# xuanyi-fu/xynet

Hardware: AMD Instinct MI355X
Metric: GiB/s device-resident WebSocket XOR-unmask, 64KiB frames, 1/2/4/8 GPUs (higher is better)
Workload: dtype u8; 1 GPU; config 3: 32768 x 64 KiB masked binary frames (H=14), one contiguous 2 GiB batch; decoder=lattice (k_stream_lattice), mode=fused (xyws_decode_stream: boundaries discovered on device), frames_per_gpu=32768, batch_bytes_per_gpu=2147942400, payload_bytes_per_gpu=2147483648, batch_copies=1, parallelism=shard-by-frame x1, no collective

## Files before the change

xynet_amd/_lib.py:

```python
import ctypes as C
import os
import re

PKG = os.path.dirname(os.path.abspath(__file__))
ROOT = os.path.dirname(PKG)
HEADER = os.path.join(ROOT, "include", "xyws.h")

XYWS_OK = 0
XYWS_ERR_DEVICE = -5
OPT_PARSE_ONLY = 0x1
OPT_UNMASKED_HINT = 0x2
OPT_SERIAL_SCAN = 0x4
OPT_WG256 = 0x8
OPT_TEST_LATSPEC = 0x10
OPT_TEST_LATDUMP = 0x20
OPT_LATX_NOWORK = 0x40
OPT_LATX_ONLY = 0x80
OPT_STATS = 0x100
OPT_SMALL_SEG = 0x200
OPT_LATTICE = 0x400
OPT_NO_LATDEC = 0x800
OPT_NO_DENSE0 = 0x1000
OPT_REDIRECT = 0x2000
OPT_NO_LATENTRY = 0x4000
OPT_WG1024 = 0x8000
OPT_RUNS_NOWAIT = 0x10000
OPT_NO_STORE = 0x20000
OPT_WG512 = 0x40000
OPT_DIAG = 0x80000
OPT_TEST_GIVEUP = 0x100000
OPT_NO_LATTICE = 0x200000
OPT_STEAL = 0x400000
OPT_TEST_STEAL = 0x800000
OPT_LAT_NOGATE = 0x1000000
OPT_LAT_GATE = 0x2000000
OPT_BIGSCAN = 0x4000000
OPT_LATX_NOCHK = 0x8000000
OPT_IOV_PIECES = 0x10000000
OPT_IOV_STAGE = 0x20000000
OPT_NO_BIGSCAN = 0x40000000
OPT_RUNS = 0x80000000
NSTATS = 48
ST_RUNS, ST_NONE, ST_BAD, ST_REPAIR, ST_CUT, ST_SPIN, ST_SEGS, ST_FRAMES = 0, 1, 2, 3, 4, 5, 6, 7
ST_P_WIN, ST_P_CAND, ST_P_UND, ST_P_TCOMP, ST_P_TCHECK, ST_P_TRES = 8, 9, 10, 11, 12, 13
ST_D_TENT, ST_D_TCHASE = 14, 15
ST_T_PRO, ST_T_MAIN, ST_T_WAIT, ST_T_FILL, ST_T_CHASE, ST_T_XOR = 16, 17, 18, 19, 20, 21
ST_T_TAIL, ST_T_PF, ST_T_CP = 22, 23, 24
ST_P_FILL, ST_P_SCAN, ST_P_PUB, ST_D_NOENT, ST_D_CHASE, ST_D_MISMATCH, ST_D_OVF = 25, 26, 27, 28, 29, 30, 31
ST_GIVEUP, ST_BRIDGE, ST_STEAL_REQ, ST_STEAL_ACC, ST_STEAL_SEGS = 32, 33, 34, 35, 36
ST_D_TVAL, ST_T_ROWS, ST_T_SER = 37, 38, 39
ST_P_LATTICE, ST_X_W0, ST_X_BITS, ST_X_SURV, ST_T_STRIDE = 40, 41, 42, 43, 46
LT_C_A, LT_C_C, LT_C_ADV, LT_D_FILL, LT_D_WB, LT_D_TAB, LT_D_WC = 16, 17, 18, 19, 20, 21, 22
LT_D_MASK, LT_D_WD, LT_D_ST, LT_D_WA, LT_SEGS, LT_GATE, LT_END = 23, 24, 25, 26, 27, 28, 29
R_WORDS = 32
R_H, R_W, R_S0, R_HEAD, R_OKW, R_HN, R_WN, R_CNT, R_TAIL, R_FIRST, R_F0 = 0, 1, 2, 7, 8, 9, 10, 11, 12, 13, 14
R_EFROM, R_ECNT, R_EORD, R_ECARRY, R_EP = 20, 21, 22, 23, 24
R_T0, R_T1, R_T2, R_SPLIT, R_XCC, R_NREC = 25, 26, 27, 28, 29, 30
POL_EPOCH, POL_BYTES, POL_FSMIN, POL_FSMAX, POL_DECODER, POL_WORDS = 0, 1, 2, 3, 4, 5
DEC_RUNS, DEC_RUNS512, DEC_LATTICE = 0, 2, 3
DERR_TABLE, DERR_TIMEOUT, DERR_STALE, DERR_TAG, DERR_SRC_OOB, DERR_ORPHANS = 0x1, 0x2, 0x4, 0x8, 0x100, 0x200
ERRORS = {-1: "invalid argument", -2: "HIP runtime error", -3: "device allocation failed",
          -4: "scratch capacity exceeded", -5: "device-side error", -6: "not complete yet"}


class XywsError(RuntimeError):
    def __init__(self, code, what=""):
        self.code = code
        super().__init__(f"xyws error {code} ({ERRORS.get(code, '?')}){': ' + what if what else ''}")


class Frame(C.Structure):
    _fields_ = [("frame_off", C.c_int64), ("payload_off", C.c_int64),
                ("payload_len", C.c_uint64), ("key", C.c_uint8 * 4),
                ("flags", C.c_uint8), ("hdr_len", C.c_uint8),
                ("status", C.c_uint8), ("reserved", C.c_uint8)]


class Carry(C.Structure):
    _fields_ = [("payload_remaining", C.c_uint64), ("phase", C.c_uint64),
                ("frames_total", C.c_uint64), ("key", C.c_uint8 * 4),
                ("hdr_len", C.c_uint8), ("hdr", C.c_uint8 * 14),
                ("reserved", C.c_uint8 * 21)]


class Verdict(C.Structure):
    _fields_ = [("close_code", C.c_uint16), ("peer_code", C.c_uint16), ("action", C.c_uint8),
                ("reserved", C.c_uint8 * 3)]


class Message(C.Structure):
    _fields_ = [("first_frame", C.c_uint64), ("nframes", C.c_uint64), ("out_off", C.c_uint64),
                ("length", C.c_uint64), ("status", C.c_uint32), ("opcode", C.c_uint8),
                ("reserved", C.c_uint8 * 3)]


class MsgCarry(C.Structure):
    _fields_ = [("length", C.c_uint64), ("nframes", C.c_uint64), ("first_frame", C.c_uint64),
                ("frame_remaining", C.c_uint64), ("frames_seen", C.c_uint64), ("status", C.c_uint32),
                ("opcode", C.c_uint8), ("frame_member", C.c_uint8), ("utf8_len", C.c_uint8),
                ("utf8", C.c_uint8 * 3), ("reserved", C.c_uint8 * 14)]


class ArenaResult(C.Structure):
    _fields_ = [("seq", C.c_uint64), ("offset", C.c_uint64), ("len", C.c_uint64), ("nframes", C.c_uint64),
                ("frames", C.POINTER(Frame)), ("carry", Carry)]


class Conn(C.Structure):
    _fields_ = [("buf", C.c_void_p), ("len", C.c_uint64), ("carry", C.c_void_p), ("frames", C.c_void_p),
                ("cap", C.c_uint64), ("reserved", C.c_uint64 * 3)]


class ReplyCarry(C.Structure):
    _fields_ = [("frame_remaining", C.c_uint64), ("frames_seen", C.c_uint64), ("replies_total", C.c_uint64),
                ("close_code", C.c_uint16), ("echoing", C.c_uint8), ("status", C.c_uint8),
                ("reserved", C.c_uint8 * 4)]


class ReplyConn(C.Structure):
    _fields_ = [("out", C.c_void_p), ("out_cap", C.c_uint64), ("rc", C.c_void_p), ("verdicts", C.c_void_p)]


class ReplyResult(C.Structure):
    _fields_ = [("reply_len", C.c_uint64), ("first_close", C.c_uint64), ("answered", C.c_uint32),
# ... 498 lines not shown
```

xynet_amd/csrc/xyws_lattice.h:

```cpp

constexpr uint64_t LAT_FMIN = 128;
constexpr uint64_t LAT_FMAX = 1ull << 40;
enum { LS_AGG = 1, LS_BRK = 3 };
constexpr uint32_t LAT_SLIST = 512;
constexpr uint32_t LAT_NOCLAIM = 0x7FFFFFFFu;
enum : uint64_t { RD_DONE = 0, RD_FULL = 1, RD_FROM = 2 };

template <uint32_t NT_, uint32_t SEG_>
struct lgeom {
  static constexpr uint32_t NT = NT_, SEG = SEG_;
  static constexpr uint32_t TMAX = SEG_ / LAT_FMIN + 3;
};
using G_LAT = lgeom<1024, 15 * 8 * 1024>;
using G_LAT5 = lgeom<1024, 15 * 5 * 1024>;
constexpr uint64_t LAT5_MIN_FRAME = 16384;
using G_LAT_SMALL = lgeom<64, 1024>;


template <class GA, class GB>
struct llay {
  static_assert(GA::NT == GB::NT, "one workgroup size");
  static constexpr uint32_t NT = GA::NT;
  static constexpr uint32_t SEG = GA::SEG > GB::SEG ? GA::SEG : GB::SEG;
  static constexpr uint32_t TMAX = GA::TMAX > GB::TMAX ? GA::TMAX : GB::TMAX;
};
template <class GL>
struct __attribute__((aligned(256))) lat_lds {
  cstate S0;
  uint64_t E, X0, F, kmax, c0, kbf, nseg;
  uint64_t gk;
  uint32_t na, cur, nxt, brk, quit, done_last, nsl, big, nogate;
  uint64_t sl_seg[LAT_SLIST], sl_k[LAT_SLIST];
  uint4 tab[GL::TMAX];
  alignas(256) uint8_t seg[GL::SEG + 48];
};

XYWS_DEV uint32_t lat_rel(uint64_t x, uint64_t ss) {
  if (x <= ss) return 0;
  const uint64_t d = x - ss;
  return d > 0xFFFFFFFFull ? 0xFFFFFFFFu : (uint32_t)d;
}

constexpr uint32_t LAT_GRP = 64;
XYWS_DEV uint64_t lat_grp_size(const run_params& P, uint64_t g) {
  const uint64_t a = g * LAT_GRP;
  return a >= P.nseg ? 0 : (P.nseg - a < LAT_GRP ? P.nseg - a : LAT_GRP);
}

XYWS_DEV uint64_t lat_advance(const run_params& P, uint64_t E, uint32_t lane) {
  const uint64_t w = uniform64(st_load(P.lat + LW_W));
  if (w >= P.nseg) return w;
  uint64_t w1 = w;
  {
    const uint64_t g0 = w / LAT_GRP, g = g0 + lane, gs = lat_grp_size(P, g);
    const bool full = !gs || st_load(P.lgrp + g) == gs;
    const uint64_t nf = __ballot(!full);
    const uint32_t c = nf ? (uint32_t)__builtin_ctzll(nf) : 64u;
    const uint64_t wg = (g0 + c) * LAT_GRP;
    if (wg > w1) w1 = wg < P.nseg ? wg : P.nseg;
  }
  if (w1 < P.nseg) {
    bool dec[4];
#pragma unroll
    for (uint32_t r = 0; r < 4; r++) {
      const uint64_t j = w1 + 4 * lane + r;
      dec[r] = j >= P.nseg || (st_load(P.lat + LW_STAT + j) >> 2) == E;
    }
    const uint32_t lc = !dec[0] ? 0u : !dec[1] ? 1u : !dec[2] ? 2u : !dec[3] ? 3u : 4u;
    const uint64_t nd = __ballot(lc < 4);
    uint64_t w2 = w1 + 256;
    if (nd) {
      const uint32_t f = (uint32_t)__builtin_ctzll(nd);
      w2 = w1 + 4 * f + (uint32_t)__shfl((int)lc, (int)f, 64);
    }
    w1 = w2 < P.nseg ? w2 : P.nseg;
  }
  if (w1 > w && lane == 0) __hip_atomic_fetch_max(P.lat + LW_W, w1, __ATOMIC_RELAXED, __HIP_MEMORY_SCOPE_AGENT);
  return w1;
}
XYWS_DEV void lat_wait_decided(const run_params& P, uint64_t E, uint64_t s, uint32_t lane) {
  for (uint32_t it = 0; lat_advance(P, E, lane) <= s; it++) {
    if (it >= (1u << 20)) {
      if (lane == 0) atomicOr(head_error(P), DERR_TIMEOUT);
      return;
    }
    __builtin_amdgcn_s_sleep(8);
  }
}

XYWS_DEV u32x4 lat_mask(const uint4* tab, uint32_t nent, uint32_t idx, uint32_t a) {
  const uint4 g = tab[idx];
  if (g.x <= a && a + 16u <= g.y) return u32x4{g.z, g.z, g.z, g.z};
  u32x4 m = span_key16(a, g.x, g.y, g.z);
  if (idx + 1 < nent) {
    const uint4 n = tab[idx + 1];
    if (n.x < a + 16u) m |= span_key16(a, n.x, n.y, n.z);
  }
  return m;
}

XYWS_DEV hdr_info lat_hdr(const run_params& P, const uint8_t* seg, uint32_t xr, uint64_t x) {
  const uint32_t* q = reinterpret_cast<const uint32_t*>(seg + (xr & ~3u));
  const uint32_t sh = xr & 3u, r0 = q[0], r1 = q[1], r2 = q[2], r3 = q[3], r4 = q[4];
  uint32_t w[4];
  w[0] = __builtin_amdgcn_alignbyte(r1, r0, sh);
  w[1] = __builtin_amdgcn_alignbyte(r2, r1, sh);
  w[2] = __builtin_amdgcn_alignbyte(r3, r2, sh);
  w[3] = __builtin_amdgcn_alignbyte(r4, r3, sh);
  const uint64_t room = P.hi - x;
  return parse_header_words(w, room < 16 ? (uint32_t)room : 16u);
}

XYWS_DEV __amdgpu_buffer_rsrc_t lat_rsrc(const run_params& P, uint64_t ss, uint32_t n) {
  const uint64_t top = (P.hi + 15) & ~15ull;
  const uint64_t room = top > ss ? top - ss : 0;
  return __builtin_amdgcn_make_buffer_rsrc(P.base + ss, 0, room < n ? (uint32_t)room : n, 0x00020000);
}

XYWS_DEV void write_frame(const run_params& P, uint64_t ord, uint64_t start, const hdr_info& h, uint64_t ps,
                          int32_t hdr_shift);

XYWS_DEV void lat_carried_frame(const run_params& P, const xyws_carry* cz) {
  if (!P.frames || !P.cap || cz->payload_remaining || !cz->hdr_len) return;
  const hdr_info hh = header_carried(P, cz);
  if (hh.hlen) write_frame(P, 0, P.lo, hh, P.lo + (hh.hlen - cz->hdr_len), (int32_t)cz->hdr_len);
}

template <class LL>
XYWS_DEV void lat_finish(const run_params& P, LL& L) {
  uint64_t* rd = P.lat + LW_REDIR;
  const xyws_carry* cz = P.cin_user ? P.cin_user : &k_zero_carry;
  {
    const uint32_t w = L.na == 2 ? LW_NBAIL_POL : L.na ? LW_NBAIL_HYP : L.big ? LW_NLOOP_A : LW_NLOOP_B;
    st_store(P.lat + w, st_load(P.lat + w) + 1);
  }
  if (L.na) {
    st_store(rd, RD_FULL);
  } else {
    const uint64_t b = st_load(P.lat + LW_BRK);
    const uint64_t X0 = L.X0, F = L.F, kmax = L.kmax, c0 = L.c0;
    lat_carried_frame(P, cz);
    if (b) {
      const uint64_t kb = ~b;
      const uint64_t tb = c0 + kb;
      uint64_t* rc = P.lat + LW_RCARRY;
#pragma unroll
      for (int i = 0; i < 8; i++) st_store(rc + i, 0);
      st_store(rc + 2, cz->frames_total + tb);
      st_store(rd + 1, X0 + kb * F);
      st_store(rd + 2, tb);
      st_store(rd, RD_FROM);
    } else {
      const uint64_t xl = X0 + (kmax - 1) * F;
      const hdr_info h = hdr_global(P, xl, NONE);
      uint64_t total = c0 + kmax;
      cstate S;
      if (!h.hlen) {
        S.X = xl; S.cov_ps = xl; S.cov_start = xl; S.cov_kw = 0; S.cov_key = 0; S.st = S_PARTIAL | S_NOCOV; S.pad = 0;
        total--;
      } else {
        S = frame_state(xl, h);
      }
      xyws_carry cinc;
#pragma unroll
      for (int i = 0; i < 8; i++) reinterpret_cast<uint64_t*>(&cinc)[i] = reinterpret_cast<const uint64_t*>(cz)[i];
      write_outputs(P, &cinc, total, S);
      dpol_publish(P, F, DEC_LATTICE);
      if (P.pol) {
        const uint64_t v[5] = {L.E, P.hi - P.lo, F, F, DEC_LATTICE};
#pragma unroll
        for (int i = 1; i < 5; i++) __hip_atomic_store(P.pol + i, v[i], __ATOMIC_RELAXED, __HIP_MEMORY_SCOPE_SYSTEM);
        __hip_atomic_store(P.pol, v[0], __ATOMIC_RELEASE, __HIP_MEMORY_SCOPE_SYSTEM);
      }
      st_store(rd, RD_DONE);
    }
  }
  uint32_t* cnt = reinterpret_cast<uint32_t*>(P.lat + LW_CNT);
  st_store(P.lat + LW_BRK, 0);
  st_store(P.lat + LW_W, 0);
  st_store(P.lat + LW_LOOPS, 0);
  __hip_atomic_store(cnt, 0u, __ATOMIC_RELAXED, __HIP_MEMORY_SCOPE_AGENT);
  __hip_atomic_store(cnt + 1, 0u, __ATOMIC_RELAXED, __HIP_MEMORY_SCOPE_AGENT);
  st_store(P.lat + LW_EPOCH, L.E);
}

XYWS_DEV bool lat_redirect(run_params& P) {
  if (!(P.opts & XYWS_OPT_REDIRECT)) return true;
  const uint64_t* r = P.lat + LW_REDIR;
  const uint64_t st = uniform64(st_load(r));
  if (st == RD_DONE) return false;
  if (st != RD_FROM) return true;
  const uint64_t p = uniform64(st_load(r + 1)), tb = uniform64(st_load(r + 2));
  const uint64_t pal = p & ~15ull;
// ... 13 lines not shown
    P.cap -= c;
  }
  return true;
}

template <class G>
struct lat_io {
  static constexpr bool CTRL = G::NT >= 256;
  static constexpr uint32_t NW = G::NT / 64, NDW = CTRL ? NW - 1 : NW;
  static constexpr uint32_t NROW = G::SEG / 1024, K = (NROW + NDW - 1) / NDW;
  static constexpr uint32_t CLAIM = CTRL ? 64u : 0u;
  static_assert(G::SEG % 1024 == 0, "segments are whole 1 KiB rows");
  XYWS_DEV static bool data_wave(uint32_t wave) { return !CTRL || wave != 0; }
  XYWS_DEV static uint32_t row(uint32_t wave, uint32_t k) { return (CTRL ? wave - 1 : wave) + NDW * k; }
  XYWS_DEV static bool valid(uint32_t wave, uint32_t k) { return K * NDW == NROW || row(wave, k) < NROW; }
};

XYWS_DEV uint64_t lat_load_late(const uint64_t* p) {
  uint64_t v;
  asm volatile("global_load_dwordx2 %0, %1, off sc1" : "=v"(v) : "v"(p) : "memory");
  return v;
}

constexpr uint32_t LAT_NREP = 64, LAT_REPW = 32;
inline constexpr uint64_t lat_rep_off(uint64_t segs) {
  return (LW_STAT + segs + segs / 64 + 1 + LAT_REPW - 1) / LAT_REPW * LAT_REPW;
}
inline constexpr uint64_t lat_sl_off(uint64_t segs) { return lat_rep_off(segs) + LAT_NREP * LAT_REPW; }
XYWS_DEV void lat_raise_brk(const run_params& P, uint64_t k, uint32_t lane) {
  uint64_t o = 0;
  if (lane == 0) o = __hip_atomic_fetch_max(P.lat + LW_BRK, ~k, __ATOMIC_RELAXED, __HIP_MEMORY_SCOPE_AGENT);
  if (uniform64(o) >= ~k) return;
  __hip_atomic_fetch_max(P.lbrk + LAT_REPW * lane, ~k, __ATOMIC_RELAXED, __HIP_MEMORY_SCOPE_AGENT);
  asm volatile("s_waitcnt vmcnt(0)" ::: "memory");
}

XYWS_DEV uint32_t lat_ctrl_load(const run_params& P, uint64_t s, uint64_t SEGB, uint64_t X0, uint64_t F, uint64_t kmax,
                                uint32_t tid) {
  const uint64_t ss = s * SEGB;
  const uint64_t ka = ss <= X0 ? 0 : (ss - X0 + F - 1) / F;
  const uint64_t xc = ka && ka <= kmax ? X0 + (ka - 1) * F : ss;
  const uint64_t top = (P.hi + 3) & ~3ull;
  const uint32_t lane = tid & 63u;
  const bool pd = lane < 4;
  uint64_t q = (pd ? ss + SEGB : xc & ~3ull) + (uint32_t)(pd ? 4u * lane : 4u * (lane - 4u));
  if (q + 4 > top) q = top - 4;
  return __builtin_nontemporal_load(reinterpret_cast<const uint32_t*>(P.base + q));
}

enum { LR_ALL = 0, LR_CTRL = 1, LR_DATA = 2 };
struct lat_clock {
  bool on;
  uint64_t t, acc[LCLK_NSLOTS];
  XYWS_DEV void start(bool o) {
    on = o;
    for (int i = 0; i < LCLK_NSLOTS; i++) acc[i] = 0;
    t = on ? __builtin_amdgcn_s_memtime() : 0;
  }
  XYWS_DEV void mark(int slot) {
    if (!on) return;
    const uint64_t n = __builtin_amdgcn_s_memtime();
    acc[slot - LCLK_SLOT0] += n - t;
    t = n;
  }
  XYWS_DEV void flush(const run_params& P) {
    if (!on) return;
    for (int i = 0; i < LCLK_NSLOTS; i++)
      if (acc[i]) stat_add(P, LCLK_SLOT0 + i, acc[i]);
  }
};
template <class G, int ROLE, class LL>
XYWS_DEV void lat_loop(const run_params& P, LL& L, uint32_t tid0, uint32_t ahead) {
  using IO = lat_io<G>;
  constexpr bool CT = ROLE != LR_DATA, DT = ROLE != LR_CTRL;
  uint32_t tid = tid0;
  asm volatile("" : "+v"(tid));
  const uint32_t lane = tid & 63u;
  const uint32_t wave = __builtin_amdgcn_readfirstlane(tid >> 6);
  uint32_t* cnt = reinterpret_cast<uint32_t*>(P.lat + LW_CNT);
  const uint64_t E = uniform64(L.E);
  const uint64_t X0 = uniform64(L.X0), F = uniform64(L.F), kmax = uniform64(L.kmax);
  const float rF = 1.0f / (float)(F < (1ull << 24) ? F : (1ull << 24));
  const uint32_t F32 = F < 0x80000000ull ? (uint32_t)F : 0x80000000u;
  uint32_t cur = uniform32(L.cur);
  uint32_t it = 0, nsl = 0;
  lat_clock clk;
  clk.start(stats_on(P) && (tid == 0 || (tid == 64 && DT)));
  uint64_t brk_seen = 0;
  const bool cl = tid == 0 && CT;
  u32x4 e[DT ? IO::K : 1];
  uint32_t cx = 0;
  constexpr uint32_t CW = IO::CLAIM / 64u;
  auto issue = [&](uint32_t s, bool claim, bool rows) {
    if constexpr (DT) {
      if (wave == CW) {
        if (lane == 0) {
          if (claim)
            asm volatile("global_atomic_add %0, %1, %2, off sc0" : "=v"(ahead) : "v"(cnt), "v"(1u) : "memory");
          else
            ahead = LAT_NOCLAIM;
        }
        cx = lat_ctrl_load(P, s, G::SEG, X0, F, kmax, tid);
      }
      if (rows) {
        const __amdgpu_buffer_rsrc_t rs = lat_rsrc(P, (uint64_t)s * G::SEG, G::SEG);
#pragma unroll
        for (uint32_t k = 0; k < IO::K; k++)
          e[k] = __builtin_amdgcn_raw_buffer_load_b128(rs, IO::valid(wave, k) ? lane * 16u : OOB,
                                                       IO::row(wave, k) * 1024u, AUX_NT);
      }
    }
  };
  if (DT && cur != NONE32) {
    const uint32_t a0 = ahead;
    issue(cur, false, true);
    ahead = a0;
    const __amdgpu_buffer_rsrc_t rs = lat_rsrc(P, (uint64_t)cur * G::SEG, G::SEG);
#pragma unroll
    for (uint32_t k = 0; k < IO::K; k++)
      __builtin_amdgcn_raw_buffer_store_b128(u32x4{0u, 0u, 0u, 0u}, rs, OOB, k * 1024u, AUX_ST_STREAM);
  }
  const uint32_t dl = IO::CTRL ? tid - 64u : tid, NDL = IO::NDW * 64u;
  while (cur != NONE32) {
    asm volatile("" : "+v"(tid));
    const uint64_t ss = (uint64_t)cur * G::SEG;
    const uint64_t se = ss + G::SEG;
    const uint64_t ka = ss <= X0 ? 0 : (ss - X0 + F - 1) / F;
    clk.mark(cl ? LT_C_ADV : LT_D_ST);
    __syncthreads();
    clk.mark(cl ? LT_C_ADV : LT_D_WA);
    if constexpr (DT) {
#pragma unroll
      for (uint32_t k = 0; k < IO::K; k++)
        if (IO::valid(wave, k)) *reinterpret_cast<u32x4*>(&L.seg[IO::row(wave, k) * 1024u + lane * 16u]) = e[k];
      if (clk.on) asm volatile("s_waitcnt lgkmcnt(0)" ::: "memory");
    }
    if (DT && wave == CW) {
      asm volatile("" : "+v"(ahead), "+v"(cx) : "v"(e[IO::K - 1].x));
      const uint32_t ln = tid & 63u;
      if (ln < 9) *reinterpret_cast<uint32_t*>(&L.seg[G::SEG + 4u * ln]) = cx;
      if (lane == 0) {
        const uint32_t a = ahead + 2u * gridDim.x;
        L.nxt = a < P.nseg ? a : NONE32;
        L.brk = NONE32;
      }
    }
    clk.mark(cl ? LT_C_A : LT_D_FILL);
    __syncthreads();
    clk.mark(cl ? LT_C_A : LT_D_WB);
    const uint32_t nxt = uniform32(L.nxt);
    uint64_t kz = se <= X0 ? 0 : (se - X0 + F - 1) / F;
    if (kz > kmax) kz = kmax;
    const uint32_t nl = kz > ka ? (uint32_t)(kz - ka) : 0u;
    if constexpr (DT) {
      if (tid == IO::CLAIM) {
        uint4 c = {0u, 0u, 0u, 0u};
        if (ka == 0) {
          const cstate S0 = L.S0;
          if (!(S0.st & S_NOCOV)) c = uint4{lat_rel(S0.cov_ps, ss), lat_rel(X0, ss), S0.cov_kw, 0u};
        } else if (ka <= kmax) {
          const uint64_t xc = X0 + (ka - 1) * F;
          const uint32_t sh = (uint32_t)(xc & 3);
          uint32_t w[4];
          const uint32_t* cw = reinterpret_cast<const uint32_t*>(&L.seg[G::SEG + 16]);
#pragma unroll
          for (int i = 0; i < 4; i++) w[i] = __builtin_amdgcn_alignbyte(cw[i + 1], cw[i], sh);
          const uint64_t room = P.hi - xc;
          const hdr_info h = parse_header_words(w, room < 16 ? (uint32_t)room : 16u);
          if (h.hlen) {
            const uint64_t ps = xc + h.hlen;
            const uint64_t end = ka == kmax ? sat_add(ps, h.plen) : xc + F;
            c = uint4{lat_rel(ps, ss), lat_rel(end < P.hi ? end : P.hi, ss), aligned_key(h.key, ps, 0), 0u};
          }
        }
        L.tab[0] = c;
      }
      if (nxt != NONE32) issue(nxt, !L.quit, true);
      const uint32_t nlw = (P.opts & XYWS_OPT_LATX_NOWORK) ? 0u : nl;
      for (uint32_t i = dl; i < nlw; i += NDL) {
        const uint64_t k = ka + i;
        const uint64_t x = X0 + k * F;
        const uint32_t xr = (uint32_t)(x - ss);
        const hdr_info h = lat_hdr(P, L.seg, xr, x);
        const bool last = k + 1 == kmax;
        const uint64_t fend = h.hlen ? sat_add(x + h.hlen, h.plen) : x;
        const bool ok = h.hlen ? ((uint64_t)h.hlen + h.plen == F && h.plen < F) || (last && fend >= P.hi) : last;
        if (!ok) atomicMin(&L.brk, i);
        uint4 en = {xr, xr, 0u, 0u};
        if (h.hlen) {
          const uint64_t ps = x + h.hlen;
          en = uint4{lat_rel(ps, ss), lat_rel(fend < P.hi ? fend : P.hi, ss), aligned_key(h.key, ps, 0), 0u};
        }
        L.tab[1 + i] = en;
      }
    }
    if (CT && tid == 0) {
      asm volatile("s_waitcnt vmcnt(0)" : "+v"(brk_seen)::"memory");
      if (cl) clk.mark(LT_GATE);
      L.gk = brk_seen;
    }
    clk.mark(cl ? LT_C_A : LT_D_TAB);
    __syncthreads();
    clk.mark(cl ? LT_C_C : LT_D_WC);
    const uint32_t brk = uniform32(L.brk);
    const bool blind = (P.opts & XYWS_OPT_TEST_LATSPEC) != 0;
    const bool gate = it == 0 && !blind && !(P.opts & XYWS_OPT_LAT_NOGATE);
    if (CT && tid < 64) {
      const uint64_t gk = uniform64(L.gk);
      if (brk != NONE32 && !(gk && ~gk <= ka + brk)) lat_raise_brk(P, ka + brk, lane);
      if (tid == 0) {
        st_store(P.lat + LW_STAT + cur, (E << 2) | (brk != NONE32 ? LS_BRK : LS_AGG));
        __hip_atomic_fetch_add(P.lgrp + cur / LAT_GRP, 1ull, __ATOMIC_RELAXED, __HIP_MEMORY_SCOPE_AGENT);
      }
      if (gate) {
        const uint64_t tg = clk.on ? __builtin_amdgcn_s_memtime() : 0;
        lat_wait_decided(P, E, cur, lane);
        if (tg && tid == 0) stat_add(P, LT_END, __builtin_amdgcn_s_memtime() - tg);
        if (tid == 0) L.gk = st_load(P.lat + LW_BRK);
      }
      if (tid == 0) brk_seen = lat_load_late(P.lbrk + LAT_REPW * (blockIdx.x % LAT_NREP));
    }
    if (gate) __syncthreads();
    clk.mark(cl ? LT_C_C : LT_D_WD);
    const uint64_t b = blind ? 0 : uniform64(L.gk);
    uint64_t kst = brk != NONE32 ? ka + brk : kz;
    if (b && ~b < kst) kst = ~b;
    uint32_t stop = kst >= kz ? G::SEG : lat_rel(X0 + kst * F, ss);
    if (stop > G::SEG) stop = G::SEG;
    bool quit = b || brk != NONE32;
    if (stop && !gate) {
      if (nsl < LAT_SLIST) {
        if (tid == IO::CLAIM) {
          L.sl_seg[nsl] = cur;
          L.sl_k[nsl] = kst;
        }
        nsl++;
      } else {
        const uint64_t k0 = ka ? ka - 1 : 0;
        if (tid == IO::CLAIM)
          for (uint32_t r = 0; r <= LAT_NREP; r++)
            __hip_atomic_fetch_max(r < LAT_NREP ? P.lbrk + LAT_REPW * r : P.lat + LW_BRK, ~k0, __ATOMIC_RELAXED,
                                   __HIP_MEMORY_SCOPE_AGENT);
        if (k0 < kst) {
          stop = lat_rel(X0 + k0 * F, ss);
          kst = k0;
        }
        quit = true;
      }
    }
    if (quit && tid == IO::CLAIM) L.quit = 1;
    if constexpr (DT) {
      const uint32_t xka = ka < kmax ? lat_rel(X0 + ka * F, ss) : 0xFFFFFFFFu;
      const uint32_t nent = brk != NONE32 ? 1u + brk : 1u + nl;
      const uint32_t lo_r = lat_rel(P.lo, ss), hi_r = P.hi - ss < G::SEG ? (uint32_t)(P.hi - ss) : G::SEG;
      const __amdgpu_buffer_rsrc_t rs = lat_rsrc(P, ss, G::SEG);
      const bool any = !(P.opts & XYWS_OPT_NO_STORE);
      const bool work = !(P.opts & XYWS_OPT_LATX_NOWORK);
      uint32_t edge = 0;
      u32x4 dprev = {0u, 0u, 0u, 0u};
#pragma unroll
      for (uint32_t k = 0; k < IO::K; k++) {
        const bool ok = IO::valid(wave, k);
        const uint32_t a = (ok ? IO::row(wave, k) : 0u) * 1024u + lane * 16u;
        u32x4 d = *reinterpret_cast<const u32x4*>(&L.seg[a]);
        uint32_t idx = 0;
        if (a >= xka) {
          const uint32_t dd = a - xka;
          uint32_t qq = (uint32_t)((float)dd * rF);
          if (qq * F32 > dd) qq--;
          else if ((qq + 1) * F32 <= dd) qq++;
          idx = 1 + qq;
        }
        if (work && idx < nent) d = d ^ lat_mask(L.tab, nent, idx, a);
        const bool whole = ok && a >= lo_r && a + 16u <= hi_r && a + 16u <= stop;
        if (ok && !whole && a < stop && a < hi_r && a + 16u > lo_r) {
          edge |= 1u << k;
          *reinterpret_cast<u32x4*>(&L.seg[a]) = d;
        }
        __builtin_amdgcn_raw_buffer_store_b128(d, rs, (whole && any) ? lane * 16u : OOB, IO::row(wave, k) * 1024u,
                                               AUX_ST_STREAM);
        asm volatile("" ::"v"(dprev.x), "v"(dprev.y), "v"(dprev.z), "v"(dprev.w));
        dprev = d;
      }
      asm volatile("s_nop 1" ::"v"(dprev.x), "v"(dprev.y), "v"(dprev.z), "v"(dprev.w));
#pragma nounroll
      while (edge && any) {
        const uint32_t k = __builtin_ctz(edge);
        edge &= edge - 1;
        const uint32_t a = IO::row(wave, k) * 1024u + lane * 16u;
#pragma nounroll
        for (uint32_t y = a; y < a + 16u; y++)
          if (y >= lo_r && y < hi_r && y < stop) P.base[ss + y] = L.seg[y];
      }
      if (P.frames && stop && kst > ka) {
        const uint32_t nd = (uint32_t)(kst - ka < nl ? kst - ka : nl);
        for (uint32_t i = dl; i < nd; i += NDL) {
          const uint64_t k = ka + i;
          const uint64_t ord = L.c0 + k;
          if (ord >= P.cap) break;
          const uint64_t x = X0 + k * F;
          const hdr_info h = lat_hdr(P, L.seg, (uint32_t)(x - ss), x);
          if (h.hlen) write_frame(P, ord, x, h, x + h.hlen, 0);
        }
      }
    }
    it++;
    if (clk.on && cl) clk.acc[LT_SEGS - LCLK_SLOT0]++;
    cur = nxt;
  }
  clk.mark(cl ? LT_C_ADV : LT_D_ST);
  clk.flush(P);
  if (DT && tid == IO::CLAIM) L.nsl = nsl;
}

constexpr uint32_t LAT_LSW = 1 + 2 * LAT_SLIST;
template <class G, class LL>
XYWS_DEV void lat_dump_list(const run_params& P, const LL& L, uint32_t tid) {
  const uint32_t n = L.nsl;
  uint64_t* q = P.lsl + (uint64_t)blockIdx.x * LAT_LSW;
  if (tid == 0) q[0] = n;
  for (uint32_t i = tid; i < n; i += G::NT) {
    q[1 + 2 * i] = L.sl_seg[i];
    q[2 + 2 * i] = L.sl_k[i];
  }
}

template <class G, class LL>
XYWS_DEV void lat_undo(const run_params& P, const LL& L, uint32_t tid, uint64_t s, uint64_t kst, uint64_t kb) {
  const uint64_t X0 = L.X0, F = L.F, kmax = L.kmax;
  const uint64_t ss = s * G::SEG;
  const uint32_t stop = (uint32_t)(X0 + kst * F - ss < G::SEG ? X0 + kst * F - ss : G::SEG);
  const uint32_t lo_r = lat_rel(P.lo, ss), hi_r = P.hi - ss < G::SEG ? (uint32_t)(P.hi - ss) : G::SEG;
  const uint32_t top = stop < hi_r ? stop : hi_r;
  const uint32_t from = lat_rel(X0 + kb * F, ss);
  for (uint32_t a = (from & ~15u) + tid * 16u; a < top; a += G::NT * 16u) {
    uint64_t g = a + ss < X0 ? NONE : (a + ss - X0) / F;
    u32x4 m = {0u, 0u, 0u, 0u};
    for (int t = 0; t < 2; t++, g = g == NONE ? 0 : g + 1) {
      uint4 en = {0u, 0u, 0u, 0u};
      if (g == NONE) {
        const cstate S0 = L.S0;
        if (!(S0.st & S_NOCOV)) en = uint4{lat_rel(S0.cov_ps, ss), lat_rel(X0, ss), S0.cov_kw, 0u};
      } else if (g < kst && g < kmax) {
        const uint64_t x = X0 + g * F;
        const hdr_info h = hdr_global(P, x, NONE);
        if (h.hlen) {
          const uint64_t ps = x + h.hlen;
          const uint64_t end = g + 1 == kmax ? sat_add(ps, h.plen) : x + F;
          en = uint4{lat_rel(ps, ss), lat_rel(end < P.hi ? end : P.hi, ss), aligned_key(h.key, ps, 0), 0u};
        }
      }
      m |= span_key16(a, en.x, en.y, en.z);
    }
    if (a >= from && a >= lo_r && a + 16u <= top) {
      uint32_t* q = reinterpret_cast<uint32_t*>(P.base + ss + a);
      const uint32_t mm[4] = {m.x, m.y, m.z, m.w};
#pragma unroll
      for (int i = 0; i < 4; i++) {
        if (!mm[i]) continue;
        const uint32_t v = __hip_atomic_load(q + i, __ATOMIC_RELAXED, __HIP_MEMORY_SCOPE_AGENT);
        __hip_atomic_store(q + i, v ^ mm[i], __ATOMIC_RELAXED, __HIP_MEMORY_SCOPE_AGENT);
      }
      continue;
    }
#pragma unroll
    for (uint32_t b = 0; b < 16; b++) {
// ... 78 lines not shown
  if (kb != NONE) {
    if (tid == 0) L.nsl = 0;
    __syncthreads();
    for (uint32_t w = tid; w < gridDim.x; w += G::NT) {
      const uint64_t* q = P.lsl + (uint64_t)w * LAT_LSW;
      const uint32_t n = (uint32_t)st_load(q);
      for (uint32_t i = 0; i < n; i++) {
        const uint64_t kst = st_load(q + 2 + 2 * i);
        if (kb < kst) {
          const uint32_t j = atomicAdd(&L.nsl, 1u);
          if (j < LAT_SLIST) {
            L.sl_seg[j] = st_load(q + 1 + 2 * i);
            L.sl_k[j] = kst;
          }
        }
      }
    }
    __syncthreads();
    const uint32_t nu = L.nsl;
    if (nu <= LAT_SLIST) {
      for (uint32_t j = 0; j < nu; j++) lat_undo<G>(P, L, tid, L.sl_seg[j], L.sl_k[j], kb);
    } else {
      for (uint32_t w = 0; w < gridDim.x; w++) {
        const uint64_t* q = P.lsl + (uint64_t)w * LAT_LSW;
        const uint32_t n = (uint32_t)st_load(q);
        for (uint32_t i = 0; i < n; i++) {
          const uint64_t kst = st_load(q + 2 + 2 * i);
          if (kb < kst) lat_undo<G>(P, L, tid, st_load(q + 1 + 2 * i), kst, kb);
        }
      }
    }
    asm volatile("s_waitcnt vmcnt(0)" ::: "memory");
    __syncthreads();
  }
  for (uint64_t g = tid; g * LAT_GRP < P.nseg; g += G::NT)
    __hip_atomic_store(P.lgrp + g, 0ull, __ATOMIC_RELAXED, __HIP_MEMORY_SCOPE_AGENT);
  if (tid < LAT_NREP) __hip_atomic_store(P.lbrk + LAT_REPW * tid, 0ull, __ATOMIC_RELAXED, __HIP_MEMORY_SCOPE_AGENT);
  if (tid != 0) return;
  lat_finish(P, L);
}

template <class GA, class GB>
__global__ void __launch_bounds__(GB::NT)
__attribute__((amdgpu_waves_per_eu(GB::NT >= 256 ? GB::NT / 256 : 1))) k_stream_lattice(run_params P0) {
  using GL = llay<GA, GB>;
  using IO = lat_io<GB>;
  static_assert(lat_io<GA>::CLAIM == IO::CLAIM, "one claim lane");
  extern __shared__ __attribute__((aligned(256))) uint8_t xs_lds[];
  lat_lds<GL>& L = *reinterpret_cast<lat_lds<GL>*>(xs_lds);
  const uint32_t tid = threadIdx.x;
  uint32_t ahead = NONE32;
  if (tid == 0) {
    const xyws_carry* cz = P0.cin_user ? P0.cin_user : &k_zero_carry;
    carry_words cc;
    uint32_t r0[5];
    uint64_t dp, ep;
    {
      u32x4 g;
      asm volatile("global_load_dwordx4 %0, %1, off sc1" : "=v"(g) : "v"(P0.lat + LW_DPOL) : "memory");
#pragma unroll
      for (int i = 0; i < 8; i++) cc.w[i] = reinterpret_cast<const uint64_t*>(cz)[i];
      const uint64_t a0 = P0.lo & ~3ull, dl = (P0.hi + 3) & ~3ull;
#pragma unroll
      for (int i = 0; i < 5; i++) {
        const uint64_t q = a0 + 4 * i;
        r0[i] = *reinterpret_cast<const uint32_t*>(P0.base + (q < dl ? q : dl - 4));
      }
      asm volatile("s_waitcnt vmcnt(0)" : "+v"(g)::"memory");
#pragma unroll
      for (int i = 0; i < 5; i++)
        if (a0 + 4 * i >= dl) r0[i] = 0u;
      dp = (uint64_t)g.x | ((uint64_t)g.y << 32);
      ep = (uint64_t)g.z | ((uint64_t)g.w << 32);
    }
    L.E = ep + 1;
    const bool dvalid = dp >> 63, dreg = (dp & ((1ull << 48) - 1)) >= LAT_FMIN;
    const uint64_t ddec = (dp >> 48) & 0x7Fu;
    uint32_t na = dvalid && !dreg && !(P0.opts & XYWS_OPT_LATTICE) ? 2u : 0u;
    L.nogate = dvalid && dreg && ddec == DEC_LATTICE && !(P0.opts & XYWS_OPT_LAT_GATE) ? 1u : 0u;
    uint64_t c0 = 0;
    const cstate S0 = initial_state_w(P0, cc, c0);
    if (!na && ((S0.st & S_PARTIAL) || S0.X >= P0.hi)) na = 1u;
    uint64_t F = 0, kmax = 0;
    if (!na) {
      hdr_info h;
      if (S0.X == P0.lo) {
        const uint32_t sh = (uint32_t)(P0.lo & 3);
        uint32_t w[4];
#pragma unroll
        for (int i = 0; i < 4; i++) w[i] = __builtin_amdgcn_alignbyte(r0[i + 1], r0[i], sh);
        const uint64_t room = P0.hi - P0.lo;
        h = parse_header_words(w, room < 16 ? (uint32_t)room : 16u);
      } else {
        h = hdr_global(P0, S0.X, NONE);
      }
      F = sat_add(h.hlen, h.plen);
      if (!h.hlen || F < LAT_FMIN || F > LAT_FMAX) na = 1;
      else kmax = (P0.hi - S0.X + F - 1) / F;
    }
    if (!na && kmax > 1 && !(P0.opts & (XYWS_OPT_TEST_LATSPEC | XYWS_OPT_LATX_NOCHK))) {
      const uint64_t dl = (P0.hi + 3) & ~3ull;
      uint32_t r[2][5];
#pragma unroll
      for (int j = 0; j < 2; j++) {
        const uint64_t a = (S0.X + (j + 1) * F) & ~3ull;
#pragma unroll
        for (int i = 0; i < 5; i++) {
          const uint64_t q = a + 4 * i;
          r[j][i] = (j == 0 || kmax > 2) && q < dl ? *reinterpret_cast<const uint32_t*>(P0.base + q) : 0u;
        }
      }
#pragma unroll
      for (int j = 0; j < 2; j++) {
        const uint64_t k = j + 1;
        if (k >= kmax) break;
        const uint64_t x = S0.X + k * F;
        const uint32_t sh = (uint32_t)(x & 3);
        uint32_t w[4];
#pragma unroll
        for (int i = 0; i < 4; i++) w[i] = __builtin_amdgcn_alignbyte(r[j][i + 1], r[j][i], sh);
        const uint64_t room = P0.hi - x;
        const hdr_info h = parse_header_words(w, room < 16 ? (uint32_t)room : 16u);
        const bool last = k + 1 == kmax;
        const uint64_t fend = h.hlen ? sat_add(x + h.hlen, h.plen) : x;
        const bool ok = h.hlen ? ((uint64_t)h.hlen + h.plen == F && h.plen < F) || (last && fend >= P0.hi) : last;
        if (!ok) na = 1;
      }
    }
    const bool big = GA::SEG != GB::SEG && !na && F >= LAT5_MIN_FRAME;
    const uint64_t seg = big ? GA::SEG : GB::SEG;
    const uint64_t nseg = (P0.hi + seg - 1) / seg;
    L.nseg = nseg;
    L.S0 = S0;
    L.c0 = c0;
    L.X0 = S0.X;
    L.F = F;
    L.kmax = kmax;
    L.na = na;
    L.quit = 0;
    L.nsl = 0;
    L.big = big ? 1u : 0u;
    L.cur = !na && blockIdx.x < nseg ? blockIdx.x : NONE32;
  }
  if (tid == IO::CLAIM) ahead = blockIdx.x - gridDim.x;
  __syncthreads();
  run_params P = P0;
  P.nseg = uniform64(L.nseg);
  P.opts &= ~XYWS_OPT_LAT_NOGATE;
  if (uniform32(L.nogate)) P.opts |= XYWS_OPT_LAT_NOGATE;
  if constexpr (GA::SEG != GB::SEG) {
    if (uniform32(L.big)) {
      lat_body<GA>(P, L, tid, ahead);
      return;
    }
  }
  lat_body<GB>(P, L, tid, ahead);
}
```

xynet_amd/csrc/xyws_stream.h:

```cpp
#pragma once
#include <hip/hip_runtime.h>
#include <stdint.h>
#include "xyws.h"
#include "xyws_host.h"


constexpr uint32_t HEAD_TICKET = 0;
constexpr uint32_t HEAD_ERROR = 4;
constexpr uint32_t HEAD_TOTAL = 8;
constexpr uint32_t HEAD_EPOCH = 16;
constexpr uint32_t HEAD_CARRY = 64;
constexpr uint32_t HEAD_STATS = 128;
constexpr uint32_t XYWS_NSTATS = 48;
constexpr uint32_t HW_DONE = 512;
constexpr uint32_t HW_BAD = 520;
constexpr uint32_t HW_TOTAL = 528;
constexpr uint32_t HW_FINAL = 536;
constexpr uint32_t HW_EMIT_SLOW = 584;
constexpr uint32_t HW_EMIT_FLAG = 592;
constexpr uint32_t HW_FSMAX = 600;
constexpr uint32_t HW_FSMIN = 608;
constexpr uint32_t HW_DPOL = 616;
constexpr uint32_t HEAD_BYTES = 1024;
static_assert(HEAD_CARRY + 64 <= HEAD_STATS && HEAD_STATS + 8 * XYWS_NSTATS <= HW_DONE, "head areas overlap");
// ... 116 lines not shown
  ST_D_OVF = 31,
  ST_GIVEUP = 32,
  ST_BRIDGE = 33,
  ST_STEAL_REQ = 34,
  ST_STEAL_ACC = 35,
  ST_STEAL_SEGS = 36,
  ST_D_TVAL = 37,
  ST_T_ROWS = 38,
  ST_T_SER = 39,
  ST_P_LATTICE = 40,
  ST_X_W0 = 41,
  ST_X_BITS = 42,
  ST_X_SURV = 43,
  ST_T_STRIDE = 46
};
enum {
  LCLK_SLOT0 = 16,
  LCLK_NSLOTS = 16
};
static_assert(LT_C_A == LCLK_SLOT0 && LT_END < LCLK_SLOT0 + LCLK_NSLOTS && LCLK_SLOT0 + LCLK_NSLOTS <= ST_GIVEUP,
              "the lattice's clocks stay in the shared slots");
static_assert(ST_T_STRIDE < XYWS_NSTATS, "a stats slot outside the head's stats area");

enum {
  POL_EPOCH = 0,
  POL_BYTES = 1,
  POL_FSMIN = 2,
  POL_FSMAX = 3,
  POL_DECODER = 4,
  POL_WORDS = 5
};
enum : uint64_t {
  DEC_RUNS = 0,
  DEC_RUNS512 = 2,
  DEC_LATTICE = 3
};

constexpr uint64_t SCRATCH_MIN_RUNS = 64, SCRATCH_MIN_SEGS = 64;
struct stream_scratch {
  xyws_internal::dev_area runs;
  int ncu = 256;
  xyws_internal::dev_area desc;
  volatile uint64_t* pol_h = nullptr;
  uint64_t* pol_d = nullptr;
  xyws_internal::dev_area lat;
};

void stream_scratch_init(stream_scratch* s, int device);
void stream_scratch_free(stream_scratch* s);
int stream_scratch_reserve(stream_scratch* s, uint64_t max_batch_bytes, uint64_t max_frames);
uint32_t stream_scratch_error(stream_scratch* s, bool clear);
int stream_scratch_stats(stream_scratch* s, uint64_t out[XYWS_NSTATS]);
int64_t stream_scratch_records(stream_scratch* s, uint64_t* out, uint64_t max_runs);
int stream_scratch_lattice(stream_scratch* s, uint64_t out[5]);
int stream_scratch_unmask_counter(stream_scratch* s, bool capturing, uint32_t** out);

#define XYWS_OPT_WG256 0x8u
#define XYWS_OPT_TEST_LATSPEC 0x10u
#define XYWS_OPT_TEST_LATDUMP 0x20u
#define XYWS_OPT_LATX_NOWORK 0x40u
#define XYWS_OPT_LATX_ONLY 0x80u
#define XYWS_OPT_STATS 0x100u
#define XYWS_OPT_SMALL_SEG 0x200u
#define XYWS_OPT_LATTICE 0x400u
#define XYWS_OPT_NO_LATDEC 0x800u
#define XYWS_OPT_NO_DENSE0 0x1000u
#define XYWS_OPT_REDIRECT 0x2000u
#define XYWS_OPT_NO_LATENTRY 0x4000u
#define XYWS_OPT_WG1024 0x8000u
#define XYWS_OPT_RUNS_NOWAIT 0x10000u
#define XYWS_OPT_NO_STORE 0x20000u
#define XYWS_OPT_WG512 0x40000u
#define XYWS_OPT_DIAG 0x80000u
#define XYWS_OPT_TEST_GIVEUP 0x100000u
#define XYWS_OPT_NO_LATTICE 0x200000u
#define XYWS_OPT_STEAL 0x400000u
#define XYWS_OPT_TEST_STEAL 0x800000u
#define XYWS_OPT_LAT_NOGATE 0x1000000u
#define XYWS_OPT_LAT_GATE 0x2000000u
#define XYWS_OPT_BIGSCAN 0x4000000u
#define XYWS_OPT_LATX_NOCHK 0x8000000u
#define XYWS_OPT_IOV_PIECES 0x10000000u
#define XYWS_OPT_IOV_STAGE 0x20000000u
#define XYWS_OPT_NO_BIGSCAN 0x40000000u
#define XYWS_OPT_RUNS 0x80000000u


struct policy_view {
  bool present;
  uint64_t epoch;
  uint64_t fsmin, fsmax;
};
policy_view policy_snapshot(const stream_scratch* s);

struct scratch_need {
  uint64_t runs;
  uint64_t fmem_bytes;
  uint64_t lat_segs;
};
inline void need_max(scratch_need* a, const scratch_need& b) {
  if (b.runs > a->runs) a->runs = b.runs;
  if (b.fmem_bytes > a->fmem_bytes) a->fmem_bytes = b.fmem_bytes;
  if (b.lat_segs > a->lat_segs) a->lat_segs = b.lat_segs;
}

enum run_geom : uint32_t { GEOM_SMALL, GEOM_MID, GEOM_WG512, GEOM_PROD };
struct decode_plan {
  uint64_t lo, hi;
  uint32_t opts;
  run_geom geom;
  uint32_t seg, threads;
  uint64_t nruns, rbytes;
  uint32_t nflat;
  bool want_lat;
  uint64_t lnseg;
  uint32_t lgrid, lseg[2];
  uint64_t pfs;
  uint32_t dense0, bigscan;
  uint64_t rcap;
  scratch_need need;
};
decode_plan plan_decode(int ncu, const policy_view& pv, uint64_t lo, uint64_t hi, uint64_t cap_if_frames,
                        uint32_t opts);
scratch_need plan_reserve(int ncu, uint64_t max_batch_bytes, uint64_t max_frames);
int reserve_for(stream_scratch* s, const scratch_need& need, bool capturing);
int launch_plan(const stream_scratch* s, const decode_plan& pl, uint8_t* base, const xyws_carry* cin,
                xyws_carry* cout, xyws_frame* frames, uint64_t cap, uint64_t* nframes, hipStream_t stream);
int stream_decode_fused(stream_scratch* s, uint8_t* base, uint64_t lo, uint64_t hi,
                        const xyws_carry* cin, xyws_carry* cout, xyws_frame* frames, uint64_t cap,
                        uint64_t* nframes, uint32_t opts, hipStream_t stream);
```

Before: 3087 GiB/s.

## Add fast plain-shape path for uniform frame headers in lattice decoder

Derives the expected header byte pattern (length and opcode bytes, excluding mask key) from the first frame. Each lattice entry whose header matches that shape gets its table entry built from the key alone, skipping full header parsing. When every frame in a segment matches, the XOR row loop uses an incremental frame-index/remainder walk and a wave-uniform fast path that applies a single key without per-row float division or span-mask work. This adds register pressure and a second unrolled loop variant. The path can be disabled with a combined option bit.

```diff
diff --git a/xynet_amd/_lib.py b/xynet_amd/_lib.py
--- a/xynet_amd/_lib.py
+++ b/xynet_amd/_lib.py
@@ -40,6 +40,7 @@
 OPT_IOV_STAGE = 0x20000000
 OPT_NO_BIGSCAN = 0x40000000
 OPT_RUNS = 0x80000000
+LATX_GENERAL = OPT_IOV_PIECES | OPT_IOV_STAGE
 NSTATS = 48
 ST_RUNS, ST_NONE, ST_BAD, ST_REPAIR, ST_CUT, ST_SPIN, ST_SEGS, ST_FRAMES = 0, 1, 2, 3, 4, 5, 6, 7
 ST_P_WIN, ST_P_CAND, ST_P_UND, ST_P_TCOMP, ST_P_TCHECK, ST_P_TRES = 8, 9, 10, 11, 12, 13
diff --git a/xynet_amd/csrc/xyws_lattice.h b/xynet_amd/csrc/xyws_lattice.h
--- a/xynet_amd/csrc/xyws_lattice.h
+++ b/xynet_amd/csrc/xyws_lattice.h
@@ -15,6 +15,37 @@
 using G_LAT5 = lgeom<1024, 15 * 5 * 1024>;
 constexpr uint64_t LAT5_MIN_FRAME = 16384;
 using G_LAT_SMALL = lgeom<64, 1024>;
+
+struct lat_shape {
+  uint32_t H, m[3], p[3];
+};
+XYWS_DEV lat_shape lat_shape_of(const hdr_info& h, uint64_t F, uint32_t opts) {
+  lat_shape s = {0u, {0u, 0u, 0u}, {0u, 0u, 0u}};
+  if (!(h.flags & XYWS_FLAG_HAS_MASK) || h.hlen < 6 || F >= (1ull << 23) ||
+      (opts & XYWS_OPT_LATX_GENERAL) == XYWS_OPT_LATX_GENERAL)
+    return s;
+  const uint32_t ext = h.hlen - 6u;
+  const uint64_t be = ext == 8   ? __builtin_bswap64(h.plen)
+                      : ext == 2 ? (((h.plen >> 8) & 0xFFull) | ((h.plen & 0xFFull) << 8))
+                                 : 0ull;
+  const uint32_t l7 = ext == 8 ? 127u : ext == 2 ? 126u : (uint32_t)h.plen;
+  s.H = h.hlen;
+  s.m[0] = ext ? 0xFFFFFF00u : 0x0000FF00u;
+  s.m[1] = ext == 8 ? 0xFFFFFFFFu : 0u;
+  s.m[2] = ext == 8 ? 0x0000FFFFu : 0u;
+  s.p[0] = ((0x80u | l7) << 8) | ((uint32_t)(be & 0xFFFFull) << 16);
+  s.p[1] = (uint32_t)(be >> 16) & s.m[1];
+  s.p[2] = (uint32_t)(be >> 48) & s.m[2];
+  return s;
+}
+XYWS_DEV bool lat_shape_match(const lat_shape& s, const uint32_t w[4]) {
+  return s.H && (((w[0] ^ s.p[0]) & s.m[0]) | ((w[1] ^ s.p[1]) & s.m[1]) | ((w[2] ^ s.p[2]) & s.m[2])) == 0u;
+}
+XYWS_DEV uint32_t lat_shape_key(uint32_t H, const uint32_t w[4]) {
+  return H == 6   ? __builtin_amdgcn_alignbyte(w[1], w[0], 2)
+         : H == 8 ? w[1]
+                  : __builtin_amdgcn_alignbyte(w[3], w[2], 2);
+}
 
 
 template <class GA, class GB>
@@ -30,6 +61,8 @@
   uint64_t E, X0, F, kmax, c0, kbf, nseg;
   uint64_t gk;
   uint32_t na, cur, nxt, brk, quit, done_last, nsl, big, nogate;
+  lat_shape shape;
+  uint32_t plain;
   uint64_t sl_seg[LAT_SLIST], sl_k[LAT_SLIST];
   uint4 tab[GL::TMAX];
   alignas(256) uint8_t seg[GL::SEG + 48];
@@ -99,16 +132,39 @@
   return m;
 }
 
-XYWS_DEV hdr_info lat_hdr(const run_params& P, const uint8_t* seg, uint32_t xr, uint64_t x) {
+XYWS_DEV u32x4 lat_mask_plain(uint32_t rem, uint32_t H, uint32_t F, uint32_t k0, uint32_t k1) {
+  const bool nx = rem + 16u > F;
+  const int32_t u = (int32_t)rem - (nx ? (int32_t)F : 0);
+  const int32_t c0 = -u, c1 = (int32_t)H - u;
+  const uint32_t z0 = (uint32_t)(c0 < 0 ? 0 : c0 > 16 ? 16 : c0);
+  const uint32_t z1 = (uint32_t)(c1 < 0 ? 0 : c1 > 16 ? 16 : c1);
+  const uint32_t kb = nx ? k1 : k0;
+  const uint32_t a0 = 4u * (z0 < 8u ? z0 : 8u), a1 = 4u * ((z0 > 8u ? z0 : 8u) - 8u);
+  const uint32_t b0 = 4u * (z1 < 8u ? z1 : 8u), b1 = 4u * ((z1 > 8u ? z1 : 8u) - 8u);
+  const uint64_t one = ~0ull;
+  const uint64_t x0 = (one << a0) << a0, x1 = (one << a1) << a1;
+  const uint64_t y0 = (one << b0) << b0, y1 = (one << b1) << b1;
+  const uint64_t K0 = (uint64_t)k0 | ((uint64_t)k0 << 32), KB = (uint64_t)kb | ((uint64_t)kb << 32);
+  const uint64_t m0 = (~x0 & K0) | (y0 & KB), m1 = (~x1 & K0) | (y1 & KB);
+  return u32x4{(uint32_t)m0, (uint32_t)(m0 >> 32), (uint32_t)m1, (uint32_t)(m1 >> 32)};
+}
+
+XYWS_DEV void lat_words(const uint8_t* seg, uint32_t xr, uint32_t w[4]) {
   const uint32_t* q = reinterpret_cast<const uint32_t*>(seg + (xr & ~3u));
   const uint32_t sh = xr & 3u, r0 = q[0], r1 = q[1], r2 = q[2], r3 = q[3], r4 = q[4];
-  uint32_t w[4];
   w[0] = __builtin_amdgcn_alignbyte(r1, r0, sh);
   w[1] = __builtin_amdgcn_alignbyte(r2, r1, sh);
   w[2] = __builtin_amdgcn_alignbyte(r3, r2, sh);
   w[3] = __builtin_amdgcn_alignbyte(r4, r3, sh);
+}
+XYWS_DEV hdr_info lat_hdr_words(const run_params& P, const uint32_t w[4], uint64_t x) {
   const uint64_t room = P.hi - x;
   return parse_header_words(w, room < 16 ? (uint32_t)room : 16u);
+}
+XYWS_DEV hdr_info lat_hdr(const run_params& P, const uint8_t* seg, uint32_t xr, uint64_t x) {
+  uint32_t w[4];
+  lat_words(seg, xr, w);
+  return lat_hdr_words(P, w, x);
 }
 
 XYWS_DEV __amdgpu_buffer_rsrc_t lat_rsrc(const run_params& P, uint64_t ss, uint32_t n) {
@@ -288,6 +344,14 @@
   const uint64_t X0 = uniform64(L.X0), F = uniform64(L.F), kmax = uniform64(L.kmax);
   const float rF = 1.0f / (float)(F < (1ull << 24) ? F : (1ull << 24));
   const uint32_t F32 = F < 0x80000000ull ? (uint32_t)F : 0x80000000u;
+  lat_shape shp;
+  shp.H = uniform32(L.shape.H);
+#pragma unroll
+  for (int i = 0; i < 3; i++) {
+    shp.m[i] = uniform32(L.shape.m[i]);
+    shp.p[i] = uniform32(L.shape.p[i]);
+  }
+  const uint32_t rstep_q = IO::NDW * 1024u / F32, rstep_r = IO::NDW * 1024u % F32;
   uint32_t cur = uniform32(L.cur);
   uint32_t it = 0, nsl = 0;
   lat_clock clk;
@@ -349,6 +413,7 @@
         const uint32_t a = ahead + 2u * gridDim.x;
         L.nxt = a < P.nseg ? a : NONE32;
         L.brk = NONE32;
+        L.plain = 1u;
       }
     }
     clk.mark(cl ? LT_C_A : LT_D_FILL);
@@ -361,6 +426,7 @@
     if constexpr (DT) {
       if (tid == IO::CLAIM) {
         uint4 c = {0u, 0u, 0u, 0u};
+        bool cplain = false;
         if (ka == 0) {
           const cstate S0 = L.S0;
           if (!(S0.st & S_NOCOV)) c = uint4{lat_rel(S0.cov_ps, ss), lat_rel(X0, ss), S0.cov_kw, 0u};
@@ -378,8 +444,10 @@
             const uint64_t end = ka == kmax ? sat_add(ps, h.plen) : xc + F;
             c = uint4{lat_rel(ps, ss), lat_rel(end < P.hi ? end : P.hi, ss), aligned_key(h.key, ps, 0), 0u};
           }
+          cplain = ka < kmax && lat_shape_match(shp, w);
         }
         L.tab[0] = c;
+        if (!cplain) L.plain = 0u;
       }
       if (nxt != NONE32) issue(nxt, !L.quit, true);
       const uint32_t nlw = (P.opts & XYWS_OPT_LATX_NOWORK) ? 0u : nl;
@@ -387,8 +455,15 @@
         const uint64_t k = ka + i;
         const uint64_t x = X0 + k * F;
         const uint32_t xr = (uint32_t)(x - ss);
-        const hdr_info h = lat_hdr(P, L.seg, xr, x);
+        uint32_t w[4];
+        lat_words(L.seg, xr, w);
         const bool last = k + 1 == kmax;
+        if (!last && lat_shape_match(shp, w)) {
+          L.tab[1 + i] = uint4{xr + shp.H, xr + F32, aligned_key(lat_shape_key(shp.H, w), x + shp.H, 0), 0u};
+          continue;
+        }
+        L.plain = 0u;
+        const hdr_info h = lat_hdr_words(P, w, x);
         const uint64_t fend = h.hlen ? sat_add(x + h.hlen, h.plen) : x;
         const bool ok = h.hlen ? ((uint64_t)h.hlen + h.plen == F && h.plen < F) || (last && fend >= P.hi) : last;
         if (!ok) atomicMin(&L.brk, i);
@@ -409,6 +484,7 @@
     __syncthreads();
     clk.mark(cl ? LT_C_C : LT_D_WC);
     const uint32_t brk = uniform32(L.brk);
+    const bool plain = DT && uniform32(L.plain) && brk == NONE32;
     const bool blind = (P.opts & XYWS_OPT_TEST_LATSPEC) != 0;
     const bool gate = it == 0 && !blind && !(P.opts & XYWS_OPT_LAT_NOGATE);
     if (CT && tid < 64) {
@@ -464,12 +540,40 @@
       const bool work = !(P.opts & XYWS_OPT_LATX_NOWORK);
       uint32_t edge = 0;
       u32x4 dprev = {0u, 0u, 0u, 0u};
+      uint32_t pidx = 0, prem = 0;
+      if (plain) {
+        const uint32_t p = IO::row(wave, 0) * 1024u + lane * 16u + (F32 - xka);
+        pidx = (uint32_t)((float)p * rF);
+        uint32_t qf = __umul24(pidx, F32);
+        const bool dn = qf > p, up = !dn && qf + F32 <= p;
+        pidx += up ? 1u : dn ? ~0u : 0u;
+        qf += up ? F32 : dn ? 0u - F32 : 0u;
+        prem = p - qf;
+      }
+      auto rows = [&](auto PL) {
+      constexpr bool PLAIN = decltype(PL)::value;
 #pragma unroll
       for (uint32_t k = 0; k < IO::K; k++) {
         const bool ok = IO::valid(wave, k);
         const uint32_t a = (ok ? IO::row(wave, k) : 0u) * 1024u + lane * 16u;
         u32x4 d = *reinterpret_cast<const u32x4*>(&L.seg[a]);
         uint32_t idx = 0;
+        if constexpr (PLAIN) {
+          const uint32_t rem = prem;
+          idx = pidx;
+          if (k + 1 < IO::K) {
+            const bool w = prem + rstep_r >= F32;
+            prem += rstep_r - (w ? F32 : 0u);
+            pidx += rstep_q + (w ? 1u : 0u);
+          }
+          if (work) {
+            const uint32_t k0 = L.tab[idx].z, k1 = L.tab[idx + 1].z;
+            if (__builtin_amdgcn_ballot_w64(rem < shp.H || rem + 16u > F32))
+              d = d ^ lat_mask_plain(rem, shp.H, F32, k0, k1);
+            else
+              d = d ^ u32x4{k0, k0, k0, k0};
+          }
+        } else {
         if (a >= xka) {
           const uint32_t dd = a - xka;
           uint32_t qq = (uint32_t)((float)dd * rF);
@@ -478,6 +582,7 @@
           idx = 1 + qq;
         }
         if (work && idx < nent) d = d ^ lat_mask(L.tab, nent, idx, a);
+        }
         const bool whole = ok && a >= lo_r && a + 16u <= hi_r && a + 16u <= stop;
         if (ok && !whole && a < stop && a < hi_r && a + 16u > lo_r) {
           edge |= 1u << k;
@@ -488,6 +593,11 @@
         asm volatile("" ::"v"(dprev.x), "v"(dprev.y), "v"(dprev.z), "v"(dprev.w));
         dprev = d;
       }
+      };
+      if (plain)
+        rows(std::true_type{});
+      else
+        rows(std::false_type{});
       asm volatile("s_nop 1" ::"v"(dprev.x), "v"(dprev.y), "v"(dprev.z), "v"(dprev.w));
 #pragma nounroll
       while (edge && any) {
@@ -732,6 +842,7 @@
     const cstate S0 = initial_state_w(P0, cc, c0);
     if (!na && ((S0.st & S_PARTIAL) || S0.X >= P0.hi)) na = 1u;
     uint64_t F = 0, kmax = 0;
+    lat_shape shape = {0u, {0u, 0u, 0u}, {0u, 0u, 0u}};
     if (!na) {
       hdr_info h;
       if (S0.X == P0.lo) {
@@ -747,6 +858,7 @@
       F = sat_add(h.hlen, h.plen);
       if (!h.hlen || F < LAT_FMIN || F > LAT_FMAX) na = 1;
       else kmax = (P0.hi - S0.X + F - 1) / F;
+      if (!na) shape = lat_shape_of(h, F, P0.opts);
     }
     if (!na && kmax > 1 && !(P0.opts & (XYWS_OPT_TEST_LATSPEC | XYWS_OPT_LATX_NOCHK))) {
       const uint64_t dl = (P0.hi + 3) & ~3ull;
@@ -790,6 +902,7 @@
     L.quit = 0;
     L.nsl = 0;
     L.big = big ? 1u : 0u;
+    L.shape = shape;
     L.cur = !na && blockIdx.x < nseg ? blockIdx.x : NONE32;
   }
   if (tid == IO::CLAIM) ahead = blockIdx.x - gridDim.x;
diff --git a/xynet_amd/csrc/xyws_stream.h b/xynet_amd/csrc/xyws_stream.h
--- a/xynet_amd/csrc/xyws_stream.h
+++ b/xynet_amd/csrc/xyws_stream.h
@@ -222,6 +222,7 @@
 #define XYWS_OPT_LATX_NOCHK 0x8000000u
 #define XYWS_OPT_IOV_PIECES 0x10000000u
 #define XYWS_OPT_IOV_STAGE 0x20000000u
+#define XYWS_OPT_LATX_GENERAL (XYWS_OPT_IOV_PIECES | XYWS_OPT_IOV_STAGE)
 #define XYWS_OPT_NO_BIGSCAN 0x40000000u
 #define XYWS_OPT_RUNS 0x80000000u
 
```

Result: no change. 3104 GiB/s, median of 6 (+0.5%).
